# jorr3/Alphazero-4-player-chess

Measured on AMD Instinct MI355X. Metric: MCTS simulations/sec (whole node), 256 games×400 sims, 10-block ResNet, higher is better.
Workload: dtype fp16

## Files before the change

alphazero-4-player-chess_amd/csrc/fpc_engine.cpp:

```cpp
#include "fpc_tree_kernels.h"

#include <algorithm>
#include <cmath>
#include <cstdarg>
#include <cstdio>
#include <cstring>
#include <string>
#include <unordered_map>
#include <vector>

#ifndef FPC_EMUL
#include <dlfcn.h>

#include "fpc_nn.h"
#endif

using namespace fpc;

namespace {
std::string g_create_error;

struct Timer {
  hipEvent_t a = nullptr, b = nullptr;
};
}

struct fpc_engine {
  fpc_config cfg{};
  DevCfg dc{};
  std::string err;
  hipStream_t stream = nullptr;
  int cap_boards = 0;
  fpc_board *d_boards = nullptr, *d_boards2 = nullptr;
  fpc_move *d_moves = nullptr;
  int *d_counts = nullptr, *d_results = nullptr, *d_err = nullptr, *d_player = nullptr, *d_flat = nullptr;
  float *d_dense = nullptr;
  Tree t{};
  std::vector<void *> allocs;
  int G = 0;
  double Cpuct = 0;
  bool searching = false;
  double *d_logtab = nullptr;
  float *d_enc_f32 = nullptr;
  float *d_stats = nullptr;
  fpc_board *d_roots = nullptr;
  int *d_rc_i = nullptr;
  float *d_rc_f = nullptr;
  double *d_rc_d = nullptr;
  int *d_rc_meta = nullptr;
  size_t rc_cap = 0;
  long sims_issued = 0;
  int leaves = 1;
  double vl = 1.0;
  int *d_VL = nullptr;
  bool stepping = false;
  bool multi = false;
  int rows_k = 1;
  bool pending_vl = false;
  fpc_tuple *d_tuples = nullptr;
  int tuple_cap = 0, tuple_count = 0;
  int *d_tgame = nullptr;
  float *d_tz = nullptr;
  float *d_noise = nullptr;
  int noise_n = 0;
  void *comm = nullptr;
  int comm_rank = 0, comm_world = 1;
  fpc_tuple *d_gather = nullptr;
  long long *d_gcounts = nullptr;
  long long comm_epoch = 0;
  int comm_fault = 0;
  int gcounts_world = 0;
  int gather_stride = 0;
  size_t gather_cap = 0;
  std::vector<int> gather_counts;
  bool timing = false;
  int policy_mode = 0;
  fpc_stats stats{};
  static constexpr int TIMING_PERIOD = 16;
  uint64_t tstep = 0;
  bool tsample = false;
  std::vector<hipEvent_t> evpool;
  std::vector<int> evtag;
  size_t evused = 0;
#ifndef FPC_EMUL
  fpc::NN nn;
#endif
};

namespace {

int fail(fpc_engine *e, int code, const char *fmt, ...) {
  char buf[512];
  va_list ap;
  va_start(ap, fmt);
  vsnprintf(buf, sizeof(buf), fmt, ap);
  va_end(ap);
  if (e) e->err = buf; else g_create_error = buf;
  return code;
}

#define USE_DEV(e)                                                                             \
  do {                                                                                         \
    if ((e) && hipSetDevice((e)->cfg.device) != hipSuccess) return fail(e, FPC_ENODEVICE, "hipSetDevice(%d) failed", (e)->cfg.device); \
  } while (0)

#define HIPCHK(e, call)                                                                        \
  do {                                                                                         \
    hipError_t _r = (call);                                                                    \
    if (_r != hipSuccess) return fail(e, FPC_ENODEVICE, "%s failed: %s", #call, hipGetErrorString(_r)); \
  } while (0)

template <class T>
int dalloc(fpc_engine *e, T **p, size_t count) {
  void *q = nullptr;
  if (hipMalloc(&q, count * sizeof(T)) != hipSuccess || !q) return fail(e, FPC_ENOMEM, "hipMalloc of %zu bytes failed", count * sizeof(T));
  if (hipMemset(q, 0, count * sizeof(T)) != hipSuccess) return fail(e, FPC_ENODEVICE, "hipMemset failed");
  e->allocs.push_back(q);
  *p = (T *)q;
  return 0;
}

int ensure_board_scratch(fpc_engine *e, int n) {
  if (n <= e->cap_boards) return 0;
  int cap = std::max(n, std::max(64, e->cap_boards * 2));
  auto re = [&](auto **p, size_t count) -> int {
    if (*p) { (void)hipFree(*p); e->allocs.erase(std::find(e->allocs.begin(), e->allocs.end(), (void *)*p)); *p = nullptr; }
    return dalloc(e, p, count);
  };
  int r;
  if ((r = re(&e->d_boards, cap))) return r;
  if ((r = re(&e->d_boards2, cap))) return r;
  if ((r = re(&e->d_moves, (size_t)cap * FPC_MAX_MOVES))) return r;
  if ((r = re(&e->d_counts, cap))) return r;
  if ((r = re(&e->d_results, cap))) return r;
  if ((r = re(&e->d_err, cap))) return r;
  if ((r = re(&e->d_player, cap))) return r;
  if ((r = re(&e->d_flat, cap))) return r;
  if ((r = re(&e->d_dense, (size_t)cap * std::max(24 * e->dc.RR, e->dc.A)))) return r;
  e->cap_boards = cap;
  return 0;
}
// ... 86 lines not shown
int fpc_action_space_size(int R) { return (8 * R + 8) * R * R; }
int fpc_is_legal_location(int R, int INV, int row, int col) {
  const int mx = R - 1;
  if (row < 0 || row > mx || col < 0 || col > mx) return 0;
  const bool cc = col < INV || col > mx - INV;
  return !(cc && (row < INV || row > mx - INV));
}
int fpc_move_flat_index(int R, int from, int to) {
  if (from < 0 || to < 0 || from >= R * R || to >= R * R || from == to) return -1;
  const int dy = to / R - from / R, dx = to % R - from % R;
  const int ay = std::abs(dy), ax = std::abs(dx);
  const bool queen = dx == 0 || dy == 0 || ax == ay;
  const bool knight = (ax == 1 && ay == 2) || (ax == 2 && ay == 1);
  if (!queen && !knight) return -1;
  DevCfg c = make_devcfg(R, 0, 0);
  return move_plane(c, from, to) * R * R + from;
}
int fpc_flat_to_move(int R, int flat, int *from, int *to) {
  DevCfg c = make_devcfg(R, 0, 0);
  if (flat < 0 || flat >= c.A) return FPC_EINVAL;
  *to = flat_to(c, flat, from);
  return 0;
}

int fpc_board_from_dict(fpc_board *out, int R, int turn, const uint8_t *sq, const uint8_t *piece, int n,
                        const uint8_t *castle4) {
  if (!out || R < 4 || R * R > FPC_MAX_SQ || turn < 0 || turn > 3 || n < 0) return FPC_EINVAL;
  memset(out, 0, sizeof(*out));
  for (int c = 0; c < 4; ++c) out->king[c] = FPC_NO_SQ;
  out->turn = (uint8_t)turn;
  if (castle4) for (int c = 0; c < 4; ++c) out->castle[c] = castle4[c] & 3;
  std::unordered_map<uint8_t, uint8_t, LocHash> m(0, LocHash{R});
  m.reserve((size_t)n);
  for (int i = 0; i < n; ++i) {
    if (sq[i] >= R * R || !(piece[i] & 0x80)) return FPC_EINVAL;
    m.emplace(sq[i], piece[i]);
  }
  std::vector<std::pair<uint8_t, uint8_t>> lists[4];
  for (const auto &it : m) {
    out->sq[it.first] = it.second;
    const int col = (it.second >> 5) & 3;
    lists[col].push_back({it.first, it.second});
    if (((it.second >> 2) & 7) == KING) out->king[col] = it.first;
  }
  static const int score[8] = {1, 2, 3, 4, 5, 0, 0, 0};
  for (int c = 0; c < 4; ++c) {
    std::sort(lists[c].begin(), lists[c].end(), [](const std::pair<uint8_t, uint8_t> &a, const std::pair<uint8_t, uint8_t> &b) {
      return score[(a.second >> 2) & 7] < score[(b.second >> 2) & 7];
    });
    if (lists[c].size() > FPC_MAX_PL) return FPC_ECAPACITY;
    out->plen[c] = (uint8_t)lists[c].size();
    for (size_t i = 0; i < lists[c].size(); ++i) out->pl[c][i] = lists[c][i].first;
  }
  return 0;
}

int fpc_board_heuristic(const fpc_board *b, int team) {
  static const int val[8] = {1, 3, 3, 5, 9, 0, 0, 0};
  int h = 0;
  for (int c = 0; c < 4; ++c)
    for (int i = 0; i < b->plen[c] && i < FPC_MAX_PL; ++i) {
      const uint8_t p = b->sq[b->pl[c][i]];
      if (!(p & 0x80)) continue;
      const int ty = (p >> 2) & 7;
      if (ty == KING) continue;
      h += (((p >> 5) & 1) == team) ? val[ty] : -val[ty];
    }
  return h;
}

int fpc_create(const fpc_config *cfg, fpc_engine **out) {
  if (!cfg || !out) return fail(nullptr, FPC_EINVAL, "null argument");
  const int R = cfg->board_size, INV = cfg->invalid_area;
  if (R < 8 || R > 14 || INV < 1 || INV > 3 || 2 * INV >= R) return fail(nullptr, FPC_EINVAL, "unsupported board %dx%d/%d (supported: 8..14 a side, cut corners 1..3)", R, R, INV);
  if (cfg->max_games < 1 || cfg->max_sims < 1) return fail(nullptr, FPC_EINVAL, "max_games/max_sims must be positive");
  int ndev = 0;
  if (hipGetDeviceCount(&ndev) != hipSuccess || ndev <= cfg->device || cfg->device < 0)
    return fail(nullptr, FPC_ENODEVICE, "no HIP device %d (found %d): this engine has no CPU path", cfg->device, ndev);
  if (hipSetDevice(cfg->device) != hipSuccess) return fail(nullptr, FPC_ENODEVICE, "hipSetDevice(%d) failed", cfg->device);
  fpc_engine *e = new fpc_engine();
  e->cfg = *cfg;
  if (e->cfg.avg_children <= 0) e->cfg.avg_children = 96;
  e->dc = make_devcfg(R, INV, FPC_RULES_STRICT);
  int r = 0;
  auto bail = [&](int code) { g_create_error = e->err; fpc_destroy(e); return code; };
  if (hipStreamCreate(&e->stream) != hipSuccess) { e->err = "hipStreamCreate failed"; return bail(FPC_ENODEVICE); }
  const int Gm = cfg->max_games;
  Tree &t = e->t;
  t.node_cap = 1 + cfg->max_sims * e->cfg.avg_children;
  t.board_cap = cfg->max_sims + 2;
  t.path_cap = cfg->max_sims + 2;
  const size_t nn = (size_t)Gm * t.node_cap;
  if ((r = dalloc(e, &t.N, nn)) || (r = dalloc(e, &t.W, nn)) || (r = dalloc(e, &t.P, nn)) || (r = dalloc(e, &t.mv, nn)) ||
      (r = dalloc(e, &t.parent, nn)) || (r = dalloc(e, &t.child0, nn)) || (r = dalloc(e, &t.nch, nn)) ||
      (r = dalloc(e, &t.bslot, nn)) || (r = dalloc(e, &t.boards, (size_t)Gm * t.board_cap)) ||
      (r = dalloc(e, &t.nnodes, Gm)) || (r = dalloc(e, &t.nboards, Gm)) || (r = dalloc(e, &t.alive, Gm)) ||
      (r = dalloc(e, &t.sims_done, Gm)) || (r = dalloc(e, &t.err, Gm)) || (r = dalloc(e, &t.leaf_node, Gm)) || (r = dalloc(e, &t.leaf_node_nx, Gm)) ||
      (r = dalloc(e, &t.leaf_slot_nx, Gm)) || (r = dalloc(e, &t.leaf_turn_nx, Gm)) ||
      (r = dalloc(e, &t.leaf_turn, Gm)) || (r = dalloc(e, &t.nlegal, Gm)) ||
      (r = dalloc(e, &t.path, (size_t)Gm * t.path_cap)) || (r = dalloc(e, &t.path_len, Gm)) ||
      (r = dalloc(e, &t.legal, (size_t)Gm * FPC_MAX_MOVES)) || (r = dalloc(e, &t.leaf_slot, Gm)) ||
      (r = dalloc(e, &e->d_enc_f32, (size_t)Gm * 24 * e->dc.RR)) || (r = dalloc(e, &e->d_stats, (size_t)Gm * SM_MAXCH * SM_REC)) || (r = dalloc(e, &e->d_roots, Gm)) ||
      (r = dalloc(e, &e->d_logtab, (size_t)cfg->max_sims + 16)) ||
      (r = dalloc(e, &e->d_rc_meta, (size_t)Gm * 3)))
    return bail(r);
  {
    std::vector<double> lt((size_t)cfg->max_sims + 16);
    for (size_t i = 0; i < lt.size(); ++i) lt[i] = i == 0 ? 0.0 : std::log(std::sqrt((double)i));
    if (hipMemcpy(e->d_logtab, lt.data(), lt.size() * sizeof(double), hipMemcpyHostToDevice) != hipSuccess) {
      e->err = "logtab upload failed";
      return bail(FPC_ENODEVICE);
    }
  }
#ifndef FPC_EMUL
  if ((r = e->nn.init(e->dc, Gm, cfg->nn_dtype, e->stream, &e->err))) return bail(r);
#endif
  *out = e;
  return 0;
}

void fpc_destroy(fpc_engine *e) {
  if (!e) return;
  (void)hipSetDevice(e->cfg.device);
  (void)fpc_comm_destroy(e);
#ifndef FPC_EMUL
  e->nn.destroy();
#endif
  for (void *p : e->allocs) (void)hipFree(p);
  for (auto &ev : e->evpool) if (ev) (void)hipEventDestroy(ev);
  if (e->stream) (void)hipStreamDestroy(e->stream);
  delete e;
}

int fpc_boards_legal_moves(fpc_engine *e, fpc_board *boards, int n, fpc_move *moves, int *counts) {
  if (!e || !boards || !moves || !counts || n < 0) return fail(e, FPC_EINVAL, "bad argument");
  USE_DEV(e);
  if (n == 0) return 0;
  int r;
  if ((r = check_boards(e, boards, n))) return r;
  if ((r = run_board_ops(e, boards, n, OP_LEGAL, nullptr, nullptr))) return r;
  HIPCHK(e, hipMemcpyAsync(boards, e->d_boards, (size_t)n * sizeof(fpc_board), hipMemcpyDeviceToHost, e->stream));
  HIPCHK(e, hipMemcpyAsync(counts, e->d_counts, (size_t)n * sizeof(int), hipMemcpyDeviceToHost, e->stream));
  HIPCHK(e, hipMemcpyAsync(moves, e->d_moves, (size_t)n * FPC_MAX_MOVES * sizeof(fpc_move), hipMemcpyDeviceToHost, e->stream));
  return fetch_errs(e, n, "board");
}

int fpc_boards_game_result(fpc_engine *e, fpc_board *boards, int n, const int *player, int *results) {
  if (!e || !boards || !results || n < 0) return fail(e, FPC_EINVAL, "bad argument");
  USE_DEV(e);
  if (n == 0) return 0;
  int r;
  if ((r = check_boards(e, boards, n))) return r;
  if ((r = run_board_ops(e, boards, n, OP_RESULT, player, nullptr))) return r;
  HIPCHK(e, hipMemcpyAsync(boards, e->d_boards, (size_t)n * sizeof(fpc_board), hipMemcpyDeviceToHost, e->stream));
  HIPCHK(e, hipMemcpyAsync(results, e->d_results, (size_t)n * sizeof(int), hipMemcpyDeviceToHost, e->stream));
  return fetch_errs(e, n, "board");
}

int fpc_boards_take_action(fpc_engine *e, const fpc_board *boards, const int *flat, int n, fpc_board *out) {
  if (!e || !boards || !flat || !out || n < 0) return fail(e, FPC_EINVAL, "bad argument");
  USE_DEV(e);
  if (n == 0) return 0;
  int r;
  if ((r = check_boards(e, boards, n))) return r;
  for (int i = 0; i < n; ++i)
    if (flat[i] < 0 || flat[i] >= e->dc.A) return fail(e, FPC_EINVAL, "flat index %d out of range", flat[i]);
// ... 36 lines not shown

int fpc_boards_legal_mask(fpc_engine *e, fpc_board *boards, int n, float *out_host) {
  if (!e || !boards || !out_host || n < 0) return fail(e, FPC_EINVAL, "bad argument");
  USE_DEV(e);
  if (n == 0) return 0;
  int r;
  if ((r = check_boards(e, boards, n))) return r;
  if ((r = run_board_ops(e, boards, n, OP_LEGAL, nullptr, nullptr))) return r;
  FPC_LAUNCH(k_mask_from_moves, n, 64, e->stream, e->dc, (const fpc_move *)e->d_moves, (const int *)e->d_counts, n, e->d_dense);
  HIPCHK(e, hipGetLastError());
  HIPCHK(e, hipMemcpyAsync(boards, e->d_boards, (size_t)n * sizeof(fpc_board), hipMemcpyDeviceToHost, e->stream));
  HIPCHK(e, hipMemcpyAsync(out_host, e->d_dense, (size_t)n * e->dc.A * sizeof(float), hipMemcpyDeviceToHost, e->stream));
  return fetch_errs(e, n, "board");
}


static int check_rows(fpc_engine *e, int leaves, int G) {
  if ((long)leaves * G > e->cfg.max_games)
    return fail(e, FPC_EINVAL, "%d leaves x %d games = %ld rows > max_games %d (fpc_search_set_leaves)", leaves, G,
                (long)leaves * G, e->cfg.max_games);
  return 0;
}

int fpc_search_begin(fpc_engine *e, const fpc_board *roots, int n_games, double c_puct) {
  if (!e || !roots || n_games < 1) return fail(e, FPC_EINVAL, "bad argument");
  USE_DEV(e);
  if (n_games > e->cfg.max_games) return fail(e, FPC_EINVAL, "n_games %d > max_games %d", n_games, e->cfg.max_games);
  int r;
  if ((r = check_rows(e, e->leaves, n_games))) return r;
  if (e->t.noise && e->noise_n != n_games)
    return fail(e, FPC_EINVAL, "root noise was uploaded for %d games, this search has %d: call fpc_search_set_root_noise again (or with NULL)", e->noise_n, n_games);
  if ((r = check_boards(e, roots, n_games))) return r;
  e->G = n_games;
  e->Cpuct = c_puct;
  HIPCHK(e, hipMemcpyAsync(e->d_roots, roots, (size_t)n_games * sizeof(fpc_board), hipMemcpyHostToDevice, e->stream));
  FPC_LAUNCH(k_search_init, n_games, 64, e->stream, e->t, n_games, (const fpc_board *)e->d_roots);
  HIPCHK(e, hipGetLastError());
  e->searching = true;
  e->sims_issued = 0;
  e->stepping = true;
  e->multi = e->leaves > 1;
  e->rows_k = 1;
  e->pending_vl = false;
  if (e->multi) {
    FPC_LAUNCH(k_vl_roots, (n_games + 63) / 64, 64, e->stream, e->d_VL, e->t.node_cap, n_games);
    HIPCHK(e, hipGetLastError());
  }
  return 0;
}

static int check_searching(fpc_engine *e) {
  return !e || !e->searching ? fail(e, FPC_ESTATE, "fpc_search_begin has not been called") : 0;
}

static int admit(fpc_engine *e, int n) {
  int r;
  if ((r = check_rows(e, e->leaves, e->G))) return r;
  if (e->sims_issued + n > e->cfg.max_sims) return fail(e, FPC_ECAPACITY, "more than max_sims = %d simulations since fpc_search_begin", e->cfg.max_sims);
  e->sims_issued += n;
  return 0;
}

static LeafPar leafpar(const fpc_engine *e) { return LeafPar{e->d_VL, e->vl}; }

static void launch_select(fpc_engine *e, int k) {
  if (e->multi)
    FPC_LAUNCH(k_select_multi, e->G, 64, e->stream, e->dc, e->t, e->G, k, e->Cpuct, (const double *)e->d_logtab, leafpar(e));
  else
    FPC_LAUNCH(k_select, e->G, 64, e->stream, e->dc, e->t, e->G, e->Cpuct, (const double *)e->d_logtab);
  e->rows_k = k;
  e->pending_vl = e->multi;
}

static void swap_leaf_arrays(fpc_engine *e) {
  std::swap(e->t.leaf_node, e->t.leaf_node_nx);
  std::swap(e->t.leaf_slot, e->t.leaf_slot_nx);
  std::swap(e->t.leaf_turn, e->t.leaf_turn_nx);
}

static void launch_expand(fpc_engine *e, const LogitSrc &src, const float *stats, const float *legal, const float *value, int ksel) {
  const int G = e->G, kexp = e->rows_k;
  const bool fuse = ksel > 0, fused = fuse && e->pending_vl == e->multi;
  const double *logtab = e->d_logtab;
  if (e->pending_vl) {
    if (legal && fuse)
      FPC_LAUNCH(k_expand_legal_select_multi, G, 64, e->stream, e->dc, e->t, G, kexp, ksel, legal, value, e->Cpuct, logtab, leafpar(e));
    else if (legal)
      FPC_LAUNCH(k_expand_legal_multi, G, 64, e->stream, e->dc, e->t, G, kexp, legal, value, leafpar(e));
    else if (fuse)
      FPC_LAUNCH(k_expand_select_multi, G, EXPAND_THREADS, e->stream, e->dc, e->t, G, kexp, ksel, src, stats, value, e->Cpuct, logtab, leafpar(e));
    else
      FPC_LAUNCH(k_expand_multi, G, EXPAND_THREADS, e->stream, e->dc, e->t, G, kexp, src, stats, value, leafpar(e));
  } else {
    if (legal && fused)
      FPC_LAUNCH(k_expand_legal_select, G, 64, e->stream, e->dc, e->t, G, legal, value, e->Cpuct, logtab);
    else if (legal)
      FPC_LAUNCH(k_expand_legal, G, 64, e->stream, e->dc, e->t, G, legal, value);
    else if (fused)
      FPC_LAUNCH(k_expand_select, G, EXPAND_THREADS, e->stream, e->dc, e->t, G, src, stats, value, e->Cpuct, logtab);
    else
      FPC_LAUNCH(k_expand, G, EXPAND_THREADS, e->stream, e->dc, e->t, G, src, stats, value);
  }
  if (fused) swap_leaf_arrays(e);
  else if (fuse) launch_select(e, ksel);
  e->rows_k = fuse ? ksel : 1;
  e->pending_vl = fuse && e->multi;
}

static void launch_partials(fpc_engine *e, const float *logits_dev) {
  const int nchunks = (e->dc.A / 4 + SM_THREADS - 1) / SM_THREADS, rows = e->rows_k * e->G;
  FPC_LAUNCH(k_softmax_partials, rows * nchunks, SM_THREADS, e->stream, logits_dev, e->dc.A, rows, nchunks, e->d_stats);
}

static int leaf_board_stride(const fpc_engine *e) { return e->pending_vl ? 0 : e->t.board_cap; }

static int finish_select(fpc_engine *e, int *n_live, const float **enc_dev) {
  const int rows = e->rows_k * e->G;
  FPC_LAUNCH(k_encode, rows, 64, e->stream, e->dc, (const fpc_board *)e->t.boards, leaf_board_stride(e),
             (const int *)e->t.leaf_slot, (const int *)e->t.leaf_turn, rows, 0, e->d_enc_f32, (uint16_t *)nullptr,
             (uint16_t)0, -1);
  HIPCHK(e, hipGetLastError());
  mark(e, 1);
  e->stats.launches_select++;
  std::vector<int> slots(rows);
  HIPCHK(e, hipMemcpyAsync(slots.data(), e->t.leaf_slot, (size_t)rows * sizeof(int), hipMemcpyDeviceToHost, e->stream));
  HIPCHK(e, hipStreamSynchronize(e->stream));
  int live = 0;
  for (int s : slots) live += s >= 0;
  if (n_live) *n_live = live;
  if (enc_dev) *enc_dev = e->d_enc_f32;
  return 0;
}

int fpc_search_select(fpc_engine *e, int *n_live, const float **enc_dev) {
  int r;
  if ((r = check_searching(e))) return r;
  USE_DEV(e);
  if ((r = admit(e, e->leaves))) return r;
  mark(e, 0);
  launch_select(e, e->leaves);
  return finish_select(e, n_live, enc_dev);
}

int fpc_search_expand_select(fpc_engine *e, const float *logits_dev, const float *value_dev, int *n_live, const float **enc_dev) {
  int r;
  if ((r = check_searching(e))) return r;
  USE_DEV(e);
  if (!logits_dev || !value_dev) return fail(e, FPC_EINVAL, "null logits/value");
  if ((r = admit(e, e->leaves))) return r;
  mark(e, 3);
  launch_partials(e, logits_dev);
  launch_expand(e, LogitSrc{logits_dev, nullptr, nullptr, 0, 0, 0, 0, 256}, e->d_stats, nullptr, value_dev, e->leaves);
  HIPCHK(e, hipGetLastError());
  mark(e, 4);
  e->stats.launches_expand++;
  mark(e, 0);
  return finish_select(e, n_live, enc_dev);
}

int fpc_search_expand(fpc_engine *e, const float *logits_dev, const float *value_dev) {
  int r;
  if ((r = check_searching(e))) return r;
  USE_DEV(e);
  if (!logits_dev || !value_dev) return fail(e, FPC_EINVAL, "null logits/value");
  mark(e, 3);
  launch_partials(e, logits_dev);
  launch_expand(e, LogitSrc{logits_dev, nullptr, nullptr, 0, 0, 0, 0, 256}, e->d_stats, nullptr, value_dev, 0);
  HIPCHK(e, hipGetLastError());
  mark(e, 4);
  e->stats.launches_expand++;
  return 0;
}

int fpc_search_set_leaves(fpc_engine *e, int leaves, double virtual_loss) {
  if (!e) return fail(e, FPC_EINVAL, "null engine");
  if (leaves < 1 || leaves > FPC_MAX_LEAVES) return fail(e, FPC_EINVAL, "leaves %d outside 1..%d", leaves, FPC_MAX_LEAVES);
  if (!std::isfinite(virtual_loss) || virtual_loss < 0.0) return fail(e, FPC_EINVAL, "virtual_loss must be finite and >= 0");
  int r;
  if (e->stepping && (r = check_rows(e, leaves, e->G))) return r;
  USE_DEV(e);
  if (leaves > 1 && !e->d_VL) {
    if ((r = dalloc(e, &e->d_VL, (size_t)e->cfg.max_games * e->t.node_cap))) return r;
  }
  if (leaves > 1 && e->searching && !e->multi) {
    HIPCHK(e, hipMemsetAsync(e->d_VL, 0, (size_t)e->cfg.max_games * e->t.node_cap * sizeof(int), e->stream));
// ... 520 lines not shown
```

alphazero-4-player-chess_amd/csrc/fpc_platform.h:

```cpp
#pragma once

#ifdef FPC_EMUL
#include "wave_emul.h"
#else
#include <hip/hip_runtime.h>
#define FPC_LAUNCH(kernel, grid, block, stream, ...) \
  hipLaunchKernelGGL(kernel, dim3(grid), dim3(block), 0, stream, __VA_ARGS__)
#endif

#include <stdint.h>

#ifdef FPC_EMUL
template <class T>
inline T wave_read(T v, int lane_uniform) { return __shfl(v, lane_uniform); }
#else
__device__ __forceinline__ int wave_read(int v, int lane_uniform) { return __builtin_amdgcn_readlane(v, lane_uniform); }
__device__ __forceinline__ float wave_read(float v, int lane_uniform) {
  return __builtin_bit_cast(float, __builtin_amdgcn_readlane(__builtin_bit_cast(int, v), lane_uniform));
}
__device__ __forceinline__ double wave_read(double v, int lane_uniform) {
  const unsigned long long b = __builtin_bit_cast(unsigned long long, v);
  const unsigned lo = (unsigned)__builtin_amdgcn_readlane((int)(unsigned)b, lane_uniform);
  const unsigned hi = (unsigned)__builtin_amdgcn_readlane((int)(unsigned)(b >> 32), lane_uniform);
  return __builtin_bit_cast(double, ((unsigned long long)hi << 32) | lo);
}
#endif
```

alphazero-4-player-chess_amd/csrc/fpc_tree_kernels.h:

```cpp
#pragma once
#include "fpc_platform.h"
#include "../../include/fpc_engine.h"

#include <type_traits>

namespace fpc {

enum { PAWN = 0, KNIGHT = 1, BISHOP = 2, ROOK = 3, QUEEN = 4, KING = 5 };

struct DevCfg {
  int R, INV, RR, A_ch, A;
  int rules;
  int rcpR;
};
__host__ __device__ __forceinline__ DevCfg make_devcfg(int R, int INV, int rules) {
  return DevCfg{R, INV, R * R, 8 * R + 8, (8 * R + 8) * R * R, rules, 65536 / R + 1};
}
__host__ __device__ __forceinline__ int row_of(const DevCfg &c, int q) { return (q * c.rcpR) >> 16; }

enum { ERR_SELECT = 1, ERR_POLICY = 2, ERR_CAP_MOVES = 4, ERR_CAP_NODES = 8, ERR_MOVE = 16, ERR_CAP_BOARDS = 32 };

struct Tree {
  int *N;
  double *W;
// ... 37 lines not shown
  int M, nlegal, first_legal, result, errbits;
  float scal_f;
};
__device__ __forceinline__ int mv_to(uint32_t w) { return (int)(w & 255u); }
__device__ __forceinline__ uint8_t mv_cap(uint32_t w) { return (uint8_t)(w >> 8); }
__device__ __forceinline__ int mv_promo(uint32_t w) { return (int)((w >> 17) & 1u); }
__device__ __forceinline__ int mv_piece(uint32_t w) { return (int)((w >> 20) & 15u); }
__device__ __forceinline__ int mv_rook(uint32_t w) { return (int)(w >> 24); }

__device__ __forceinline__ bool present(uint8_t p) { return (p & 0x80) != 0; }
__device__ __forceinline__ int colour_of(uint8_t p) { return (p >> 5) & 3; }
__device__ __forceinline__ int type_of(uint8_t p) { return (p >> 2) & 7; }
__device__ __forceinline__ int team_of_colour(int c) { return c & 1; }
__device__ __forceinline__ int team_of(uint8_t p) { return (p >> 5) & 1; }

__device__ __forceinline__ bool legal_loc(const DevCfg &c, int row, int col) {
  const int mx = c.R - 1;
  const bool in = ((unsigned)row <= (unsigned)mx) & ((unsigned)col <= (unsigned)mx);
  const bool cc = (col < c.INV) | (col > mx - c.INV);
  const bool rr = (row < c.INV) | (row > mx - c.INV);
  return in & !(cc & rr);
}
__host__ __device__ __forceinline__ bool in_array(const DevCfg &c, int row, int col) {
  return ((unsigned)row < (unsigned)c.R) & ((unsigned)col < (unsigned)c.R);
}

__host__ __device__ __forceinline__ int move_plane(const DevCfg &c, int from, int to) {
  const int fr = row_of(c, from), tr = row_of(c, to);
  const int dy = tr - fr, dx = (to - tr * c.R) - (from - fr * c.R);
  const int ay = dy < 0 ? -dy : dy, ax = dx < 0 ? -dx : dx;
  if (dx == 0 || dy == 0 || ax == ay) {
    const int sx = (dx > 0) - (dx < 0), sy = (dy > 0) - (dy < 0);
    const int key = (sx + 1) * 3 + (sy + 1);
    int dir;
    switch (key) {
      case 0: dir = 1; break; case 1: dir = 2; break; case 2: dir = 3; break;
      case 3: dir = 0; break; case 5: dir = 4; break;
      case 6: dir = 7; break; case 7: dir = 6; break; default: dir = 5; break;
    }
    const int dist = ax > ay ? ax : ay;
    return dir * (c.R - 1) + dist - 1;
  }
  const int k = (dx == -2 ? 0 : dx == -1 ? 2 : dx == 1 ? 4 : 6) + (dy > 0 ? 1 : 0);
  return 8 * (c.R - 1) + k;
}

__host__ __device__ __forceinline__ int flat_to(const DevCfg &c, int flat, int *from_out) {
  const int plane = flat / c.RR, from = flat % c.RR;
  *from_out = from;
  const int nq = c.R - 1;
  int dx, dy;
  if (plane < 8 * nq) {
    const int dir = plane / nq, dist = plane % nq + 1;
    const int qdx[8] = {0, -1, -1, -1, 0, 1, 1, 1};
    const int qdy[8] = {-1, -1, 0, 1, 1, 1, 0, -1};
    dx = qdx[dir] * dist; dy = qdy[dir] * dist;
  } else {
    const int k = plane - 8 * nq;
    if (k >= 8) return FPC_NO_SQ;
    const int ndx[8] = {-2, -2, -1, -1, 1, 1, 2, 2};
    const int ndy[8] = {-1, 1, -2, 2, -2, 2, -1, 1};
    dx = ndx[k]; dy = ndy[k];
  }
  const int row = from / c.R + dy, col = from % c.R + dx;
  if (!in_array(c, row, col)) return FPC_NO_SQ;
  return row * c.R + col;
}

__device__ __forceinline__ int piece_plane(uint8_t p, int turn, int rules) {
  int plane = 6 * ((colour_of(p) - turn) & 3) + type_of(p);
  if (!(rules & FPC_RULES_PLANES)) { plane -= 1; if (plane < 0) plane += 24; }
  return plane;
}

__device__ __forceinline__ int rot90_src(int R, int k, int i, int j) {
  k &= 3;
  return k == 0 ? i * R + j : k == 1 ? j * R + (R - 1 - i) : k == 2 ? (R - 1 - i) * R + (R - 1 - j) : (R - 1 - j) * R + i;
}

__device__ __forceinline__ int lane_id() { return (int)(threadIdx.x & 63); }

#ifdef FPC_TREE_STAMPS
__device__ unsigned long long g_tree_stamps[32];
#define FPC_TS(I) do { if ((int)blockIdx.x == FPC_TREE_STAMPS && lane_id() == 0) g_tree_stamps[I] = __builtin_amdgcn_s_memtime(); } while (0)
#else
#define FPC_TS(I) do {} while (0)
#endif

__device__ __forceinline__ void lds_load_board(WaveLds *s, const fpc_board *g) {
  const uint32_t *src = reinterpret_cast<const uint32_t *>(g);
  uint32_t *dst = reinterpret_cast<uint32_t *>(&s->b);
  const int l = lane_id();
  dst[l] = src[l];
  if (l < 8) dst[64 + l] = src[64 + l];
  __syncthreads();
}
__device__ __forceinline__ void lds_store_board(const WaveLds *s, fpc_board *g) {
  __syncthreads();
  const uint32_t *src = reinterpret_cast<const uint32_t *>(&s->b);
  uint32_t *dst = reinterpret_cast<uint32_t *>(g);
  const int l = lane_id();
  dst[l] = src[l];
  if (l < 8) dst[64 + l] = src[64 + l];
}

__device__ __forceinline__ bool promotes(const DevCfg &c, int colour, int tr, int tc) {
  switch (colour) {
    case 0: return tr == c.R / 4;
    case 1: return tc == 3 * c.R / 4;
    case 2: return tr == 3 * c.R / 4;
    default: return tc == c.R / 4;
  }
}

__device__ __forceinline__ int wave_list_erase_append(uint8_t *list, int len, int sq, int add, bool *found) {
  const int lane = lane_id();
  const int v = (lane < len && lane < FPC_MAX_PL) ? list[lane] : -1;
  const int nxt = __shfl(v, lane + 1 < 64 ? lane + 1 : lane);
  const unsigned long long hit = __ballot(v == sq);
  __syncthreads();
  const int idx = hit ? (int)__ffsll((long long)hit) - 1 : -1;
  int n = len;
  if (idx >= 0) {
    if (lane >= idx && lane + 1 < len) list[lane] = (uint8_t)nxt;
    n = len - 1;
  }
  if (add >= 0 && n < FPC_MAX_PL) { if (lane == 0) list[n] = (uint8_t)add; ++n; }
  *found = idx >= 0;
  __syncthreads();
  return n;
}

template <bool LEAF_PARALLEL = false>
__device__ inline bool make_move_wave(fpc_board *b, int from, int to, const DevCfg &c) {
  const int lane = lane_id();
  if (to == FPC_NO_SQ) return false;
  uint8_t piece = b->sq[from];
  const uint8_t cap = b->sq[to];
  bool found;
  __syncthreads();
  if (present(cap)) {
    const int cc = colour_of(cap);
    const int n = wave_list_erase_append(b->pl[cc], b->plen[cc], to, -1, &found);
    if (lane == 0) {
      b->plen[cc] = (uint8_t)n;
      b->sq[to] = 0;
      if (type_of(cap) == KING) b->king[cc] = FPC_NO_SQ;
    }
    __syncthreads();
  }
  if (!present(piece)) return false;
  const int pc = colour_of(piece);
  int rook_from = FPC_NO_SQ, rook_to = FPC_NO_SQ;
  uint8_t rights = b->castle[pc];
  if (c.rules & FPC_RULES_FULL_MOVES) {
    const int R = c.R, fr = row_of(c, from), fc = from - fr * R, tr = row_of(c, to), tc = to - tr * R;
    const int ty = type_of(piece);
    if (ty == PAWN) {
      if (promotes(c, pc, tr, tc)) piece = (uint8_t)(0x80 | (pc << 5) | (QUEEN << 2));
    } else if (ty == KING) {
      const int dr = tr - fr, dc = tc - fc;
      if ((dr == 0 && (dc == 2 || dc == -2)) || (dc == 0 && (dr == 2 || dr == -2))) {
        const int ur = dr / 2, uc = dc / 2;
        for (int d = 3; d <= 4; ++d) {
          const int rr = fr + ur * d, rc = fc + uc * d;
          if (in_array(c, rr, rc)) {
            const uint8_t rk = b->sq[rr * R + rc];
            if (present(rk) && type_of(rk) == ROOK && colour_of(rk) == pc) { rook_from = rr * R + rc; rook_to = (fr + ur) * R + fc + uc; break; }
            if (present(rk)) break;
// ... 1169 lines not shown
  }
  for (int off = 32; off >= 1; off >>= 1) part = part + __shfl_xor(part, off);
  if (lane == 0) red[wave] = part;
  __syncthreads();
  if (tid == 0) { rec[0] = m; rec[1] = ((red[0] + red[1]) + red[2]) + red[3]; rec[2] = nf; rec[3] = 0.f; }
}

__global__ void __launch_bounds__(SM_THREADS) k_softmax_partials(const float *logits, int A, int G, int nchunks, float *stats) {
  __shared__ float red[8];
  const int g = (int)blockIdx.x / nchunks, ch = (int)blockIdx.x % nchunks;
  if (g >= G) return;
  const int q = ch * SM_THREADS + (int)threadIdx.x;
  const bool valid = q * 4 < A;
  const float4 v = valid ? *reinterpret_cast<const float4 *>(logits + (size_t)g * A + 4 * q) : float4{0.f, 0.f, 0.f, 0.f};
  softmax_chunk_stats(v, valid, red, stats + ((size_t)g * SM_MAXCH + ch) * SM_REC);
}

constexpr int EXPAND_THREADS = 64;
constexpr int LOGIT_MAX_SLABS = 8;
struct LogitSrc {
  const float *dense;
  const float *part, *bias;
  int G1, s1, s2, Mtot;
  int gw;
};
__device__ __forceinline__ float logit_at(const LogitSrc &L, int g, int A, int idx) {
  if (L.dense) return L.dense[(size_t)g * A + idx];
  const int j = L.gw == 256 ? idx >> 8 : idx / L.gw, col = idx - j * L.gw;
  const int base = j < L.G1 ? j * L.s1 : L.G1 * L.s1 + (j - L.G1) * L.s2, cnt = j < L.G1 ? L.s1 : L.s2;
  float p[LOGIT_MAX_SLABS];
#pragma unroll
  for (int k = 0; k < LOGIT_MAX_SLABS; ++k) p[k] = k < cnt ? L.part[((size_t)(base + k) * L.Mtot + g) * L.gw + col] : 0.f;
  float v = L.bias[idx];
#pragma unroll
  for (int k = 0; k < LOGIT_MAX_SLABS; ++k) v = k < cnt ? v + p[k] : v;
  return v;
}
template <bool MULTI>
__device__ inline bool expand_game(WaveLds &s, const DevCfg &c, const Tree &t, int G, int g, int row, const LogitSrc &logits,
                                   const float *stats, const float *value, int *VL) {
  const int lane = lane_id();
  const size_t nb = (size_t)g * t.node_cap;
  const int nchunks = (c.A / 4 + SM_THREADS - 1) / SM_THREADS;
  const float *st = stats + (size_t)row * SM_MAXCH * SM_REC;
  const uint16_t *legal = t.legal + (size_t)row * FPC_MAX_MOVES;
  const int n = t.leaf_node[row];
  const int nl = t.nlegal[row];
  const int own_turn = t.leaf_turn[row];
  const int scan_node = lane < G ? t.leaf_node[lane] : -1;
  const int scan_turn = lane < G ? t.leaf_turn[lane] : 0;
  const int fl0 = legal[lane];
  float mc = -__builtin_inff(), sc = 0.f;
  bool nan = false;
  if (lane < nchunks) { mc = st[lane * SM_REC]; sc = st[lane * SM_REC + 1]; nan = st[lane * SM_REC + 2] != 0.f; }
  const ExpandPre pre = expand_prefetch(t, g, row, value);
  int turn0;
  if (c.rules & FPC_RULES_ROTATION) turn0 = own_turn;
  else {
    const unsigned long long bal = __ballot(scan_node >= 0);
    turn0 = bal ? wave_read(scan_turn, (int)__ffsll((long long)bal) - 1) : (G > 64 ? first_leaf_turn(t.leaf_node, t.leaf_turn, G) : 0);
  }
  if (n < 0) return true;
  FPC_TS(1);
  float m = mc;
  for (int off = 32; off >= 1; off >>= 1) { const float o = __shfl_xor(m, off); m = o > m ? o : m; }
  nan = __ballot(nan) != 0ull;
  const float term = (lane < nchunks && mc > -__builtin_inff()) ? sc * fpc_expf(mc - m) : 0.f;
  float S = 0.f;
  for (int k = 0; k < nchunks; ++k) S = S + wave_read(term, k);
  const float inv = fdiv_rn(1.0f, S);
  FPC_TS(2);
  for (int j = lane; j < nl; j += 64) {
    const int fl = j < 64 ? fl0 : (int)legal[j];
    const int plane = fl / c.RR, pos = fl % c.RR;
    const int src = plane * c.RR + rot90_src(c.R, -turn0, pos / c.R, pos % c.R);
    s.pri[j] = fpc_expf(logit_at(logits, row, c.A, src) - m) * inv;
    s.lsorted[j] = (uint16_t)fl;
  }
  __syncthreads();
  FPC_TS(3);
  return expand_finish<MULTI>(s, t, g, row, nb, n, nl, nan, pre, VL);
}

__global__ void __launch_bounds__(EXPAND_THREADS) k_expand(DevCfg c, Tree t, int G, LogitSrc logits, const float *stats, const float *value) {
  __shared__ WaveLds s;
  const int g = blockIdx.x;
  if (g >= G) return;
  (void)expand_game<false>(s, c, t, G, g, g, logits, stats, value, nullptr);
}

__global__ void __launch_bounds__(EXPAND_THREADS) k_expand_select(DevCfg c, Tree t, int G, LogitSrc logits, const float *stats,
                                                                  const float *value, double Cpuct, const double *logtab) {
  __shared__ WaveLds s;
  const int g = blockIdx.x;
  if (g >= G) return;
  FPC_TS(0);
  (void)expand_game<false>(s, c, t, G, g, g, logits, stats, value, nullptr);
  __syncthreads();
  FPC_TS(4);
  select_game(s, c, t, g, Cpuct, logtab, true, ONE_LEAF);
}


template <bool MULTI>
__device__ inline bool expand_legal_game(WaveLds &s, const DevCfg &c, const Tree &t, int g, int row, const float *ll, const float *value, int *VL) {
  const int lane = lane_id();
  const int n = t.leaf_node[row];
  const ExpandPre pre = expand_prefetch(t, g, row, value);
  if (n < 0) return true;
  const size_t nb = (size_t)g * t.node_cap;
  const int nl = t.nlegal[row];
  const uint16_t *legal = t.legal + (size_t)row * FPC_MAX_MOVES;
  const float *lg = ll + (size_t)row * FPC_MAX_MOVES;
  float m = -__builtin_inff();
  bool nan = false;
  for (int j = lane; j < nl; j += 64) { const float v = lg[j]; nan |= v != v; m = v > m ? v : m; }
  for (int off = 32; off >= 1; off >>= 1) { const float o = __shfl_xor(m, off); m = o > m ? o : m; }
  nan = __ballot(nan) != 0ull;
  for (int j = lane; j < nl; j += 64) {
    s.pri[j] = m == -__builtin_inff() ? 0.f : fpc_expf(lg[j] - m);
    s.lsorted[j] = legal[j];
  }
  __syncthreads();
  return expand_finish<MULTI>(s, t, g, row, nb, n, nl, nan, pre, VL);
}

__global__ void __launch_bounds__(64) k_expand_legal(DevCfg c, Tree t, int G, const float *ll, const float *value) {
  __shared__ WaveLds s;
  const int g = blockIdx.x;
  if (g >= G) return;
  (void)expand_legal_game<false>(s, c, t, g, g, ll, value, nullptr);
}

__global__ void __launch_bounds__(64) k_expand_legal_select(DevCfg c, Tree t, int G, const float *ll, const float *value, double Cpuct,
                                                            const double *logtab) {
  __shared__ WaveLds s;
  const int g = blockIdx.x;
  if (g >= G) return;
  (void)expand_legal_game<false>(s, c, t, g, g, ll, value, nullptr);
  __syncthreads();
  select_game(s, c, t, g, Cpuct, logtab, true, ONE_LEAF);
}

template <bool LEGAL>
__device__ inline void expand_game_multi(WaveLds &s, const DevCfg &c, const Tree &t, int G, int g, int kexp, const LogitSrc &logits,
                                         const float *ll, const float *stats, const float *value, int *VL) {
  for (int k = 0; k < kexp; ++k) {
    const int row = k * G + g;
    bool ok;
    if constexpr (LEGAL) ok = expand_legal_game<true>(s, c, t, g, row, ll, value, VL);
    else ok = expand_game<true>(s, c, t, kexp * G, g, row, logits, stats, value, VL);
    __syncthreads();
    if (!ok) break;
  }
}

__global__ void __launch_bounds__(EXPAND_THREADS) k_expand_multi(DevCfg c, Tree t, int G, int kexp, LogitSrc logits, const float *stats,
                                                                 const float *value, LeafPar lp) {
  __shared__ WaveLds s;
  const int g = blockIdx.x;
  if (g >= G) return;
  expand_game_multi<false>(s, c, t, G, g, kexp, logits, nullptr, stats, value, lp.VL);
}

__global__ void __launch_bounds__(EXPAND_THREADS) k_expand_select_multi(DevCfg c, Tree t, int G, int kexp, int ksel, LogitSrc logits,
                                                                        const float *stats, const float *value, double Cpuct,
                                                                        const double *logtab, LeafPar lp) {
  __shared__ WaveLds s;
  const int g = blockIdx.x;
  if (g >= G) return;
  expand_game_multi<false>(s, c, t, G, g, kexp, logits, nullptr, stats, value, lp.VL);
  select_game_multi(s, c, t, G, g, ksel, Cpuct, logtab, true, lp);
}

__global__ void __launch_bounds__(64) k_expand_legal_multi(DevCfg c, Tree t, int G, int kexp, const float *ll, const float *value, LeafPar lp) {
  __shared__ WaveLds s;
  const int g = blockIdx.x;
  if (g >= G) return;
  expand_game_multi<true>(s, c, t, G, g, kexp, LogitSrc{}, ll, nullptr, value, lp.VL);
}

__global__ void __launch_bounds__(64) k_expand_legal_select_multi(DevCfg c, Tree t, int G, int kexp, int ksel, const float *ll,
                                                                  const float *value, double Cpuct, const double *logtab, LeafPar lp) {
  __shared__ WaveLds s;
  const int g = blockIdx.x;
  if (g >= G) return;
  expand_game_multi<true>(s, c, t, G, g, kexp, LogitSrc{}, ll, nullptr, value, lp.VL);
  select_game_multi(s, c, t, G, g, ksel, Cpuct, logtab, true, lp);
}

}
```

Before: 492,400.

## Add helper waves that prefetch descent-path tree data during fused expand-select

The fused expand+select kernels are templated on a wave count and now launch four waves per game by default. Wave 0 does the usual expand and select work. The three extra waves walk the current leaf paths and touch node stats, child arrays, boards, log-table entries and virtual-loss counters, so these land in cache before the select descent reads them. This aims to hide the latency of the dependent global loads in tree traversal. In exchange it adds memory traffic and larger blocks that may reduce occupancy, and an env knob can turn it off.

Result: no change. 491,500 (-0.2%).

```diff
diff --git a/alphazero-4-player-chess_amd/csrc/fpc_engine.cpp b/alphazero-4-player-chess_amd/csrc/fpc_engine.cpp
--- a/alphazero-4-player-chess_amd/csrc/fpc_engine.cpp
+++ b/alphazero-4-player-chess_amd/csrc/fpc_engine.cpp
@@ -57,6 +57,7 @@
   bool multi = false;
   int rows_k = 1;
   bool pending_vl = false;
+  bool tree_helpers = true;
   fpc_tuple *d_tuples = nullptr;
   int tuple_cap = 0, tuple_count = 0;
   int *d_tgame = nullptr;
@@ -309,6 +310,8 @@
   e->cfg = *cfg;
   if (e->cfg.avg_children <= 0) e->cfg.avg_children = 96;
   e->dc = make_devcfg(R, INV, FPC_RULES_STRICT);
+  if (getenv("FPC_DEV_KNOBS") && atoi(getenv("FPC_DEV_KNOBS")) != 0 && getenv("FPC_TREE_WAVES"))
+    e->tree_helpers = atoi(getenv("FPC_TREE_WAVES")) != 1;
   int r = 0;
   auto bail = [&](int code) { g_create_error = e->err; fpc_destroy(e); return code; };
   if (hipStreamCreate(&e->stream) != hipSuccess) { e->err = "hipStreamCreate failed"; return bail(FPC_ENODEVICE); }
@@ -511,25 +514,31 @@
   const int G = e->G, kexp = e->rows_k;
   const bool fuse = ksel > 0, fused = fuse && e->pending_vl == e->multi;
   const double *logtab = e->d_logtab;
+#define FPC_LAUNCH_FUSED(kernel, ...)                                                        \
+  do {                                                                                       \
+    if (e->tree_helpers) FPC_LAUNCH(kernel<TREE_WAVES>, G, 64 * TREE_WAVES, e->stream, __VA_ARGS__); \
+    else FPC_LAUNCH(kernel<1>, G, 64, e->stream, __VA_ARGS__);                               \
+  } while (0)
   if (e->pending_vl) {
     if (legal && fuse)
-      FPC_LAUNCH(k_expand_legal_select_multi, G, 64, e->stream, e->dc, e->t, G, kexp, ksel, legal, value, e->Cpuct, logtab, leafpar(e));
+      FPC_LAUNCH_FUSED(k_expand_legal_select_multi, e->dc, e->t, G, kexp, ksel, legal, value, e->Cpuct, logtab, leafpar(e));
     else if (legal)
       FPC_LAUNCH(k_expand_legal_multi, G, 64, e->stream, e->dc, e->t, G, kexp, legal, value, leafpar(e));
     else if (fuse)
-      FPC_LAUNCH(k_expand_select_multi, G, EXPAND_THREADS, e->stream, e->dc, e->t, G, kexp, ksel, src, stats, value, e->Cpuct, logtab, leafpar(e));
+      FPC_LAUNCH_FUSED(k_expand_select_multi, e->dc, e->t, G, kexp, ksel, src, stats, value, e->Cpuct, logtab, leafpar(e));
     else
       FPC_LAUNCH(k_expand_multi, G, EXPAND_THREADS, e->stream, e->dc, e->t, G, kexp, src, stats, value, leafpar(e));
   } else {
     if (legal && fused)
-      FPC_LAUNCH(k_expand_legal_select, G, 64, e->stream, e->dc, e->t, G, legal, value, e->Cpuct, logtab);
+      FPC_LAUNCH_FUSED(k_expand_legal_select, e->dc, e->t, G, legal, value, e->Cpuct, logtab);
     else if (legal)
       FPC_LAUNCH(k_expand_legal, G, 64, e->stream, e->dc, e->t, G, legal, value);
     else if (fused)
-      FPC_LAUNCH(k_expand_select, G, EXPAND_THREADS, e->stream, e->dc, e->t, G, src, stats, value, e->Cpuct, logtab);
+      FPC_LAUNCH_FUSED(k_expand_select, e->dc, e->t, G, src, stats, value, e->Cpuct, logtab);
     else
       FPC_LAUNCH(k_expand, G, EXPAND_THREADS, e->stream, e->dc, e->t, G, src, stats, value);
   }
+#undef FPC_LAUNCH_FUSED
   if (fused) swap_leaf_arrays(e);
   else if (fuse) launch_select(e, ksel);
   e->rows_k = fuse ? ksel : 1;
diff --git a/alphazero-4-player-chess_amd/csrc/fpc_platform.h b/alphazero-4-player-chess_amd/csrc/fpc_platform.h
--- a/alphazero-4-player-chess_amd/csrc/fpc_platform.h
+++ b/alphazero-4-player-chess_amd/csrc/fpc_platform.h
@@ -25,3 +25,9 @@
   return __builtin_bit_cast(double, ((unsigned long long)hi << 32) | lo);
 }
 #endif
+
+#ifdef FPC_EMUL
+inline void consume(int v) { asm volatile("" ::"r"(v)); }
+#else
+__device__ __forceinline__ void consume(int v) { asm volatile("" ::"v"(v)); }
+#endif
diff --git a/alphazero-4-player-chess_amd/csrc/fpc_tree_kernels.h b/alphazero-4-player-chess_amd/csrc/fpc_tree_kernels.h
--- a/alphazero-4-player-chess_amd/csrc/fpc_tree_kernels.h
+++ b/alphazero-4-player-chess_amd/csrc/fpc_tree_kernels.h
@@ -143,9 +143,11 @@
 
 #ifdef FPC_TREE_STAMPS
 __device__ unsigned long long g_tree_stamps[32];
-#define FPC_TS(I) do { if ((int)blockIdx.x == FPC_TREE_STAMPS && lane_id() == 0) g_tree_stamps[I] = __builtin_amdgcn_s_memtime(); } while (0)
+#define FPC_TS(I) do { if ((int)blockIdx.x == FPC_TREE_STAMPS && threadIdx.x == 0) g_tree_stamps[I] = __builtin_amdgcn_s_memtime(); } while (0)
+#define FPC_TS_HELPER(I) do { if ((int)blockIdx.x == FPC_TREE_STAMPS && threadIdx.x == 64) g_tree_stamps[I] = __builtin_amdgcn_s_memtime(); } while (0)
 #else
 #define FPC_TS(I) do {} while (0)
+#define FPC_TS_HELPER(I) do {} while (0)
 #endif
 
 __device__ __forceinline__ void lds_load_board(WaveLds *s, const fpc_board *g) {
@@ -1481,6 +1483,67 @@
   return expand_finish<MULTI>(s, t, g, row, nb, n, nl, nan, pre, VL);
 }
 
+constexpr int TREE_WAVES = 4;
+__device__ __forceinline__ int clampi(int v, int lo, int hi) { return v < lo ? lo : (v > hi ? hi : v); }
+__device__ inline void descent_prefetch(const Tree &t, int G, int g, int krows, int hw, int nhw, const double *logtab, const int *VL) {
+  const int lane = lane_id();
+  const size_t nb = (size_t)g * t.node_cap;
+  const int nn = clampi(t.nnodes[g], 1, t.node_cap);
+  int acc = t.alive[g] ^ t.nboards[g];
+  for (int k = 0; k < krows; ++k) {
+    const int row = k * G + g;
+    const int len = clampi(t.path_len[row], 0, t.path_cap < 64 ? t.path_cap : 64);
+    const bool on = lane < len;
+    const int node = on ? clampi(t.path[(size_t)row * t.path_cap + lane], 0, nn - 1) : 0;
+    int c0 = on ? t.child0[nb + node] : -1;
+    int nc = on ? (int)t.nch[nb + node] : 0;
+    const int Nn = on ? t.N[nb + node] : 0;
+    const int bs = on ? t.bslot[nb + node] : -1;
+    if (c0 < 0 || c0 >= nn) { c0 = 0; nc = 0; }
+    nc = nc < nn - c0 ? nc : nn - c0;
+    if (on) {
+      acc ^= logtab[clampi(Nn + 1, 0, t.path_cap - 1)] > 1.0 ? 1 : 0;
+      if (bs >= 0 && bs < t.board_cap) {
+        const uint32_t *bw = reinterpret_cast<const uint32_t *>(&t.boards[(size_t)g * t.board_cap + bs]);
+        acc ^= (int)(bw[0] ^ bw[32] ^ bw[64] ^ bw[71]);
+      }
+    }
+    int incl = nc;
+    for (int off = 1; off < 64; off <<= 1) {
+      const int v = __shfl_up(incl, off);
+      if (lane >= off) incl += v;
+    }
+    const int total = wave_read(incl, 63);
+    for (int q0 = hw * 64; q0 < total; q0 += nhw * 64) {
+      const int q = q0 + lane;
+      int lv = 0;
+      for (int j = 0; j < len; ++j) lv += q >= wave_read(incl, j) ? 1 : 0;
+      lv = lv < 63 ? lv : 63;
+      const int first = __shfl(incl - nc, lv), cc0 = __shfl(c0, lv);
+      if (q < total) {
+        const size_t i = nb + cc0 + (q - first);
+        int a = t.N[i] ^ t.child0[i] ^ t.bslot[i] ^ (int)t.nch[i] ^ (int)t.mv[i];
+        a ^= t.W[i] > 0.0 ? 1 : 0;
+        a ^= t.P[i] > 0.f ? 1 : 0;
+        if (VL) a ^= VL[i];
+        acc ^= a;
+      }
+    }
+  }
+  consume(acc);
+  FPC_TS_HELPER(14);
+}
+template <int NW>
+__device__ __forceinline__ bool helper_wave_done(const Tree &t, int G, int g, int krows, const double *logtab, const int *VL) {
+  if constexpr (NW > 1) {
+    if (threadIdx.x >= 64) {
+      descent_prefetch(t, G, g, krows, (int)(threadIdx.x >> 6) - 1, NW - 1, logtab, VL);
+      return true;
+    }
+  }
+  return false;
+}
+
 __global__ void __launch_bounds__(EXPAND_THREADS) k_expand(DevCfg c, Tree t, int G, LogitSrc logits, const float *stats, const float *value) {
   __shared__ WaveLds s;
   const int g = blockIdx.x;
@@ -1488,11 +1551,13 @@
   (void)expand_game<false>(s, c, t, G, g, g, logits, stats, value, nullptr);
 }
 
-__global__ void __launch_bounds__(EXPAND_THREADS) k_expand_select(DevCfg c, Tree t, int G, LogitSrc logits, const float *stats,
-                                                                  const float *value, double Cpuct, const double *logtab) {
+template <int NW>
+__global__ void __launch_bounds__(64 * NW) k_expand_select(DevCfg c, Tree t, int G, LogitSrc logits, const float *stats,
+                                                           const float *value, double Cpuct, const double *logtab) {
   __shared__ WaveLds s;
   const int g = blockIdx.x;
   if (g >= G) return;
+  if (helper_wave_done<NW>(t, G, g, 1, logtab, nullptr)) return;
   FPC_TS(0);
   (void)expand_game<false>(s, c, t, G, g, g, logits, stats, value, nullptr);
   __syncthreads();
@@ -1531,11 +1596,13 @@
   (void)expand_legal_game<false>(s, c, t, g, g, ll, value, nullptr);
 }
 
-__global__ void __launch_bounds__(64) k_expand_legal_select(DevCfg c, Tree t, int G, const float *ll, const float *value, double Cpuct,
-                                                            const double *logtab) {
+template <int NW>
+__global__ void __launch_bounds__(64 * NW) k_expand_legal_select(DevCfg c, Tree t, int G, const float *ll, const float *value, double Cpuct,
+                                                                 const double *logtab) {
   __shared__ WaveLds s;
   const int g = blockIdx.x;
   if (g >= G) return;
+  if (helper_wave_done<NW>(t, G, g, 1, logtab, nullptr)) return;
   (void)expand_legal_game<false>(s, c, t, g, g, ll, value, nullptr);
   __syncthreads();
   select_game(s, c, t, g, Cpuct, logtab, true, ONE_LEAF);
@@ -1562,12 +1629,14 @@
   expand_game_multi<false>(s, c, t, G, g, kexp, logits, nullptr, stats, value, lp.VL);
 }
 
-__global__ void __launch_bounds__(EXPAND_THREADS) k_expand_select_multi(DevCfg c, Tree t, int G, int kexp, int ksel, LogitSrc logits,
-                                                                        const float *stats, const float *value, double Cpuct,
-                                                                        const double *logtab, LeafPar lp) {
+template <int NW>
+__global__ void __launch_bounds__(64 * NW) k_expand_select_multi(DevCfg c, Tree t, int G, int kexp, int ksel, LogitSrc logits,
+                                                                 const float *stats, const float *value, double Cpuct,
+                                                                 const double *logtab, LeafPar lp) {
   __shared__ WaveLds s;
   const int g = blockIdx.x;
   if (g >= G) return;
+  if (helper_wave_done<NW>(t, G, g, kexp, logtab, lp.VL)) return;
   expand_game_multi<false>(s, c, t, G, g, kexp, logits, nullptr, stats, value, lp.VL);
   select_game_multi(s, c, t, G, g, ksel, Cpuct, logtab, true, lp);
 }
@@ -1579,11 +1648,13 @@
   expand_game_multi<true>(s, c, t, G, g, kexp, LogitSrc{}, ll, nullptr, value, lp.VL);
 }
 
-__global__ void __launch_bounds__(64) k_expand_legal_select_multi(DevCfg c, Tree t, int G, int kexp, int ksel, const float *ll,
-                                                                  const float *value, double Cpuct, const double *logtab, LeafPar lp) {
+template <int NW>
+__global__ void __launch_bounds__(64 * NW) k_expand_legal_select_multi(DevCfg c, Tree t, int G, int kexp, int ksel, const float *ll,
+                                                                       const float *value, double Cpuct, const double *logtab, LeafPar lp) {
   __shared__ WaveLds s;
   const int g = blockIdx.x;
   if (g >= G) return;
+  if (helper_wave_done<NW>(t, G, g, kexp, logtab, lp.VL)) return;
   expand_game_multi<true>(s, c, t, G, g, kexp, LogitSrc{}, ll, nullptr, value, lp.VL);
   select_game_multi(s, c, t, G, g, ksel, Cpuct, logtab, true, lp);
 }
```
